# yumi-crew/pose_estimation

Measured on NVIDIA B200. Metric: icp_hypotheses_per_s, higher is better.
Workload: dtype f32

## Files before the change

pose_estimation_b200/csrc/api.cu:

```cuda
#include <algorithm>
#include <cstring>
#include <new>

#include "core_math.cuh"

namespace peb {

int fail(peb_ctx* ctx, int code, const char* fmt, ...) {
  char buf[512];
  va_list ap;
  va_start(ap, fmt);
  vsnprintf(buf, sizeof(buf), fmt, ap);
  va_end(ap);
  if (ctx) ctx->err = buf;
  return code;
}

namespace {

thread_local std::string g_create_error;

__global__ void __launch_bounds__(256) repack_kernel(const unsigned char* __restrict__ raw, size_t stride, int n,
                                                     float w_fill, float4* __restrict__ out) {
  const int i = blockIdx.x * blockDim.x + threadIdx.x;
// ... 202 lines not shown
  if (!strcmp(key, "source_sort_occupancy")) {
    if (value < 1 || value > 1024) return fail(ctx, PEB_E_INVALID_ARG, "source_sort_occupancy out of [1, 1024]");
    ctx->src_sort_occupancy = static_cast<float>(value);
    return PEB_OK;
  }
  if (!strcmp(key, "cert_margin_x1000")) {
    if (value < 0 || value > 4000) return fail(ctx, PEB_E_INVALID_ARG, "cert_margin_x1000 out of [0, 4000]");
    ctx->cert_margin = value / 1000.0f;
    return PEB_OK;
  }
  if (!strcmp(key, "seed_guard_x10")) {
    if (value < 0 || value > 100000) return fail(ctx, PEB_E_INVALID_ARG, "seed_guard_x10 out of [0, 100000]");
    ctx->seed_guard = value / 10.0f;
    return PEB_OK;
  }
  if (!strcmp(key, "batch_streams")) {
    if (value < 0 || value > 32) return fail(ctx, PEB_E_INVALID_ARG, "batch_streams out of [0, 32]");
    ctx->batch_streams = value;
    return PEB_OK;
  }
  if (!strcmp(key, "blocks_factor")) {
    if (value < 0 || value > 4096) return fail(ctx, PEB_E_INVALID_ARG, "blocks_factor out of [0, 4096]");
    ctx->blocks_factor = value;
    return PEB_OK;
  }
  if (!strcmp(key, "coop_max_rows")) {
    if (value < 0 || value > (1 << 20)) return fail(ctx, PEB_E_INVALID_ARG, "coop_max_rows out of [0, 2^20]");
    ctx->coop_max_rows = value;
    return PEB_OK;
  }
  if (!strcmp(key, "blocks_factor_cold")) {
    if (value < 0 || value > 4096) return fail(ctx, PEB_E_INVALID_ARG, "blocks_factor_cold out of [0, 4096]");
    ctx->blocks_factor_cold = value;
    return PEB_OK;
  }
  if (!strcmp(key, "flag_deps")) {
    ctx->flag_deps = value != 0;
    return PEB_OK;
  }
  if (!strcmp(key, "pdl")) {
    ctx->use_pdl = value != 0;
    return PEB_OK;
  }
  if (!strcmp(key, "debug_timers")) {
    ctx->debug_timers = value != 0;
    return PEB_OK;
  }
  if (!strcmp(key, "anchor_seed")) {
    ctx->anchor_seed = value != 0;
    return PEB_OK;
  }
  if (!strcmp(key, "warm_start")) {
    ctx->warm_start = value != 0;
    return PEB_OK;
  }
  if (!strcmp(key, "warm_graph")) {
    if (value < 0 || value > 1) return fail(ctx, PEB_E_INVALID_ARG, "warm_graph must be 0 or 1");
    ctx->warm_graph = value;
    return PEB_OK;
  }
  if (!strcmp(key, "warm_graph_kappa_x100")) {
    if (value < 0 || value > 100000) return fail(ctx, PEB_E_INVALID_ARG, "warm_graph_kappa_x100 out of [0, 100000]");
    ctx->warm_graph_kappa = value / 100.0f;
    return PEB_OK;
  }
  if (!strcmp(key, "warm_graph_queue")) {
// ... 669 lines not shown
```

pose_estimation_b200/csrc/common.cuh:

```cuda
#pragma once

#include <cuda_runtime.h>

#include <cstdarg>
#include <cstdint>
#include <cstdio>
#include <string>
#include <vector>

#include "../../include/pe_b200.h"

#define PEB_HD __host__ __device__ __forceinline__

namespace peb {

constexpr int kSmCount = 148;

struct DevBuf {
  void* p = nullptr;
  size_t cap = 0;
  cudaError_t ensure(size_t bytes) {
    if (bytes <= cap) return cudaSuccess;
    if (p) cudaFree(p);
    p = nullptr;
// ... 56 lines not shown
  bool valid = false;
};

}

struct peb_ctx {
  int device = 0;
  cudaStream_t stream = nullptr;
  std::string err;
  uint64_t launches = 0;
  int nn_group = 1;
  float grid_occupancy = 5.0f;
  bool warm_start = true;
  int warm_upfront = 0;
  int warm_upfront_from = 2;
  int warm_graph = 1;
  float warm_graph_kappa = 0.0f;
  int warm_graph_queue = 0;
  int warm_graph_flat = 1;
  int warm_graph_flat_from = 2, warm_graph_flat_until = 15;
  int warm_graph_peek = 1;
  int cold_graph = 1;
  int warm_graph_min_hyp = 32;
  int warm_bin = 0;
  bool anchor_seed = true;
  int coop_max_rows = 1024;
  float seed_guard = 10.0f;
  int batch_streams = 0;
  std::vector<cudaStream_t> sub_streams;
  std::vector<cudaEvent_t> join_events;
  cudaEvent_t fork_event = nullptr;
  int blocks_factor = 0;
  int blocks_factor_cold = 0;
  bool flag_deps = true;
  peb::DevBuf epochs;
  int* last_err_flag = nullptr;
  bool use_pdl = true;
  bool debug_timers = false;
  peb::DevBuf dbg;
  int dbg_launches = 0;
  peb::DevBuf anchors;
  int nn_cache_from = 0;
  float nn_cache_r = 0.75f;
  peb::DevBuf nn_cache;
  float cert_margin = 0.0f;

  peb::PinnedBuf h_stage;
  peb::PinnedBuf h_small;
  peb::DevBuf d_small;
  peb::DevBuf d_scratch;
  peb::DevBuf sort_scratch;
  peb::DevBuf scan_scratch[4];
  peb::DevBuf d_stage;

  peb::DevBuf tgt_raw;
  peb::DevBuf tgt_nrm_raw;
  size_t n_tgt = 0;
  bool tgt_has_normals = false;
  bool tgt_staged = false;
  cudaEvent_t tgt_stage_event = nullptr;
  peb::Grid tgt_grid;
  peb::DevBuf tgt_knn;
  peb::DevBuf tgt_knn_aux;
  peb::DevBuf tgt_knn_stat;
  bool tgt_knn_valid = false;

// ... 105 lines not shown
```

pose_estimation_b200/csrc/core_math.cuh:

```cuda
#pragma once

#include <cfloat>
#include <cmath>

#include "common.cuh"

namespace peb {

struct Mat4 {
  float m[16];
};

PEB_HD Mat4 mat4_identity() {
  Mat4 a;
#pragma unroll
  for (int i = 0; i < 16; ++i) a.m[i] = (i % 5 == 0) ? 1.0f : 0.0f;
  return a;
}

PEB_HD Mat4 mat4_mul(const Mat4& a, const Mat4& b) {
  Mat4 r;
#pragma unroll
  for (int j = 0; j < 4; ++j)
#pragma unroll
// ... 579 lines not shown
  for (int r = 5; r >= 0; --r) {
    double v = b[r];
    for (int c = r + 1; c < 6; ++c) v -= A[r * 6 + c] * x[c];
    x[r] = v / A[r * 6 + r];
  }
  const double alpha = x[0], beta = x[1], gamma = x[2];
  const double ca = cos(alpha), sa = sin(alpha), cb = cos(beta), sb = sin(beta), cg = cos(gamma), sg = sin(gamma);
  Mat4 T;
  for (int i = 0; i < 16; ++i) T.m[i] = 0.0f;
  T.m[0] = static_cast<float>(cg * cb);
  T.m[4] = static_cast<float>(-sg * ca + cg * sb * sa);
  T.m[8] = static_cast<float>(sg * sa + cg * sb * ca);
  T.m[1] = static_cast<float>(sg * cb);
  T.m[5] = static_cast<float>(cg * ca + sg * sb * sa);
  T.m[9] = static_cast<float>(-cg * sa + sg * sb * ca);
  T.m[2] = static_cast<float>(-sb);
  T.m[6] = static_cast<float>(cb * sa);
  T.m[10] = static_cast<float>(cb * ca);
  T.m[12] = static_cast<float>(x[3]);
  T.m[13] = static_cast<float>(x[4]);
  T.m[14] = static_cast<float>(x[5]);
  T.m[15] = 1.0f;
  return T;
}

struct IcpState {
  Mat4 inc;
  Mat4 final_t;
  double prev_mse, cur_mse;
  double fit_sum;
  int iterations, state, converged, similar;
  int ncorr, active, fit_n, pad0;
  unsigned ticket, ticket_fit;
  int pad1[2];
};

struct IcpCriteria {
  int max_iterations, min_correspondences, max_similar, estimator;
  double rotation_threshold, translation_threshold, mse_rel, mse_abs;
};

PEB_HD void icp_finish_iteration_scripted(IcpState& st, const IcpCriteria& cr, const Mat4& inc, double sum_d2, int n) {
  st.ncorr = n;
  if (n < cr.min_correspondences) {
    st.state = PEB_NO_CORRESPONDENCES;
    st.converged = 0;
    st.active = 0;
    return;
  }
  st.inc = inc;
  st.final_t = mat4_mul(st.inc, st.final_t);
  st.iterations += 1;
  bool is_similar = false;
  bool ret = false;
  int state = PEB_NOT_CONVERGED;
  const float* t = st.inc.m;
  do {
    if (st.iterations >= cr.max_iterations) {
      state = PEB_ITERATIONS;
      ret = true;
      break;
    }
    double cos_angle = 0.5 * static_cast<double>(t[0] + t[5] + t[10] - 1.0f);
    double translation_sqr = static_cast<double>(t[12] * t[12] + t[13] * t[13] + t[14] * t[14]);
    if (cos_angle >= cr.rotation_threshold && translation_sqr <= cr.translation_threshold) {
      if (st.similar >= cr.max_similar) {
        state = PEB_TRANSFORM;
// ... 171 lines not shown
```

pose_estimation_b200/csrc/icp.cu:

```cuda
#include <algorithm>

#include "nn_cache.cuh"
#include "nn_graph.cuh"
#include "nn_search.cuh"
#include "nn_upfront.cuh"

namespace peb {

namespace {

constexpr int kIcpThreads = 128;
constexpr int kMinBlocksSingle = 5;
#ifndef PEB_MIN_BLOCKS_BATCH
#define PEB_MIN_BLOCKS_BATCH 8
#endif
constexpr int kMinBlocksBatch = PEB_MIN_BLOCKS_BATCH;

struct IcpLaunch {
  GridView grid;
  const float4* src;
  float4* work;
  float* slack;
  const int* anchors;
  int n_anchor;
  float seed_guard2;
  int coop_max_rows;
  unsigned long long* dbg;
  int launch_idx;
  IcpState* states;
  double* partials;
  int part_stride;
  int32_t* corr_idx;
  float* corr_d2;
  Mat4* trace;
  peb_icp_result* results;
  IcpCriteria crit;
  double max_dist_sqr;
  double fitness_max_range;
  float stop_d2;
  float fitness_stop_d2;
  float rej_max2;
  int use_rejector;
  int n_src;
  int blocks_per_hyp;
  int trace_cap;
  int fitness_only;
  int warm;
  int* epochs;
  int* err_flag;
// ... 5 lines not shown
  const double* knn_stat;
  float knn_kappa;
  int cold_graph;
  int knn_peek_until;
  const float4* knn_aux;
};

__global__ void icp_init_kernel(IcpState* __restrict__ states, const float* __restrict__ guesses, int H,
                                int* __restrict__ epochs) {
  const int h = blockIdx.x * blockDim.x + threadIdx.x;
  if (epochs && h <= H) epochs[h] = 0;
  if (h >= H) return;
  IcpState st;
  st.inc = mat4_identity();
  if (guesses) {
#pragma unroll
    for (int i = 0; i < 16; ++i) st.final_t.m[i] = guesses[16 * h + i];
  } else {
    st.final_t = mat4_identity();
  }
  st.prev_mse = DBL_MAX;
  st.cur_mse = DBL_MAX;
  st.fit_sum = 0.0;
  st.iterations = 0;
  st.state = PEB_NOT_CONVERGED;
  st.converged = 0;
  st.similar = 0;
  st.ncorr = 0;
  st.active = 1;
  st.fit_n = 0;
  st.pad0 = 0;
  st.ticket = 0;
  st.ticket_fit = 0;
  st.pad1[0] = st.pad1[1] = 0;
  states[h] = st;
}

template <int NACC>
__device__ __forceinline__ double block_reduce_acc(double (&acc)[NACC], double (*sm)[kAccMax]) {
  const int lane = threadIdx.x & 31, warp = threadIdx.x >> 5;
#pragma unroll
  for (int i = 0; i < NACC; ++i) {
    double v = acc[i];
#pragma unroll
    for (int o = 16; o > 0; o >>= 1) v += __shfl_xor_sync(0xFFFFFFFFu, v, o);
    if (lane == 0) sm[warp][i] = v;
  }
  __syncthreads();
  double r = 0.0;
  if (threadIdx.x < NACC) {
#pragma unroll
    for (int w = 0; w < kIcpThreads / 32; ++w) r += sm[w][threadIdx.x];
  }
  return r;
}

template <int NACC>
__device__ __forceinline__ void reduce_partials(const double* __restrict__ part, int n_blocks, double (*sm)[kAccMax],
                                                double* sm_out) {
  const int lane = threadIdx.x & 31, warp = threadIdx.x >> 5;
  constexpr int kW = kIcpThreads / 32;
  double v = 0.0;
  if (lane < NACC) {
    const int per = (n_blocks + kW - 1) / kW;
    const int b0 = warp * per, b1 = min(b0 + per, n_blocks);
    const double* p = part + lane;
    int b = b0;
// ... 50 lines not shown
template <int MB>
__device__ __noinline__ void finish_iteration(IcpState* st, const IcpCriteria* cr, const double* acc, Mat4* trace,
                                              int trace_cap, unsigned long long* dbg) {
  if (dbg) dbg[5] = global_ns();
  IcpState s = *st;
  if (dbg) dbg[6] = global_ns() + (s.iterations < -5 ? 1 : 0);
  icp_finish_iteration(s, *cr, acc);
  if (dbg) dbg[7] = global_ns() + (s.iterations < -5 ? 1 : 0);
  s.ticket = 0;
  if (trace && s.state != PEB_NO_CORRESPONDENCES && s.iterations >= 1 && s.iterations <= trace_cap)
    trace[s.iterations - 1] = s.inc;
  *st = s;
}

__device__ __forceinline__ void pdl_trigger_and_wait() {
  asm volatile("griddepcontrol.launch_dependents;");
  asm volatile("griddepcontrol.wait;" ::: "memory");
}

__device__ __forceinline__ int ld_acquire_gpu(const int* p) {
  int v;
  asm volatile("ld.acquire.gpu.global.s32 %0, [%1];" : "=r"(v) : "l"(p) : "memory");
  return v;
}


constexpr int kEpochStopped = 1 << 20;
constexpr unsigned long long kFlagWaitLimitNs = 20ull * 1000ull * 1000ull * 1000ull;
__device__ __forceinline__ void wait_for_hypothesis(const int* __restrict__ solved, int need, int* err_flag) {
  if (threadIdx.x == 0 && ld_acquire_gpu(solved) < need) {
    const unsigned long long t0 = global_ns();
    unsigned spins = 0;
    while (ld_acquire_gpu(solved) < need) {
      __nanosleep(40);
      if ((++spins & 0xFFFu) == 0u && global_ns() - t0 > kFlagWaitLimitNs) {
        atomicExch(err_flag, 1);
        break;
      }
    }
  }
  __syncthreads();
}

__device__ __forceinline__ bool graph_pays(const IcpLaunch& L, const IcpState* st) {
  if (!L.knn) return false;
  if (L.knn_kappa <= 0.0f) return true;
  const double mse = __ldcg(&st->cur_mse);
  const double cnt = __ldcg(L.knn_stat + 1);
  return cnt > 0.0 && 4.0 * mse * static_cast<double>(L.knn_kappa) * cnt < __ldcg(L.knn_stat);
}

template <int EST, int NACC>
__device__ __forceinline__ void accumulate_pair_impl(const GridView& g, const float4& p, const NnBest& best,
                                                     double (&acc)[NACC]) {
  const float4 t = g.pts[best.j];
  if (EST == PEB_ESTIMATOR_SVD) {
    const double sx = p.x, sy = p.y, sz = p.z, tx = t.x, ty = t.y, tz = t.z;
    acc[0] += 1.0;
    acc[1] += sx;
    acc[2] += sy;
    acc[3] += sz;
    acc[4] += tx;
    acc[5] += ty;
    acc[6] += tz;
    acc[7] = fma(tx, sx, acc[7]);
    acc[8] = fma(tx, sy, acc[8]);
// ... 146 lines not shown
          best.d2 = l2_simple(p.x, p.y, p.z, t.x, t.y, t.z);
          best.idx = __float_as_int(t.w);
          best.j = j_prev;
        } else {
          best = grid_nn_warm_cert(L.grid, p.x, p.y, p.z, j_prev, L.stop_d2, L.margin, &slack);
        }
        *sl = slack;
      } else {
        if (UPF == 4 || UPF == 6) best = graph ? grid_nn_warm_graph(L.grid, L.knn, p.x, p.y, p.z, j_prev, L.stop_d2, kGraphSkipHopeless, L.launch_idx <= L.knn_peek_until, UPF == 6 ? L.knn_aux : nullptr)
                                   : grid_nn_warm(L.grid, p.x, p.y, p.z, j_prev, L.stop_d2);
        else best = UPF ? grid_nn_warm_upfront<(UPF == 3 ? 3 : 2)>(L.grid, p.x, p.y, p.z, j_prev, L.stop_d2)
                        : grid_nn_warm(L.grid, p.x, p.y, p.z, j_prev, L.stop_d2);
      }
    } else {
      best = grid_nn<G>(L.grid, p.x, p.y, p.z, L.stop_d2);
      if (CERT && lane_in_group == 0) *sl = -1.0f;
    }
  }
  if (in && lane_in_group == 0 && (first || valid)) {
    p.w = __int_as_float(best.j);
    work[i] = p;
  }
  bool keep = valid && best.idx >= 0;
  if (keep && static_cast<double>(best.d2) > L.max_dist_sqr) keep = false;
  if (keep && L.use_rejector && !(best.d2 < L.rej_max2)) keep = false;
  if (in && lane_in_group == 0 && L.corr_idx) {
    const int orig = __float_as_int(L.src[i].w);
    L.corr_idx[orig] = keep ? best.idx : -1;
    L.corr_d2[orig] = keep ? best.d2 : 0.0f;
  }
  if (keep && lane_in_group == 0) accumulate_pair<EST>(L.grid, p, best, acc);
}

template <int G, int EST, int MB, bool CERT, bool FIRST, int UPF>
__device__ __forceinline__ void icp_iteration_body(const IcpLaunch& L, const int h, const int blk) {
  unsigned long long t_dbg[5];
  if (L.dbg) t_dbg[0] = global_ns();
  constexpr int NACC = (EST == PEB_ESTIMATOR_SVD) ? kAccSvd : kAccLls;
  __shared__ double sm[kIcpThreads / 32][kAccMax];
  __shared__ double sm_tot[kAccMax];
  __shared__ float s_inc[16];
  __shared__ int s_flags[4];
  __shared__ CoopTile s_tile[kIcpThreads / 32];
  IcpState* st = L.states + h;
  if (threadIdx.x < 16) s_inc[threadIdx.x] = FIRST ? __ldcg(&st->final_t.m[threadIdx.x]) : __ldcg(&st->inc.m[threadIdx.x]);
  if (threadIdx.x == 32) {
    const int active = __ldcg(&st->active);
    const int first = FIRST ? 1 : 0;
    int apply = 1;
    if (first) {
      apply = 0;
      for (int i = 0; i < 16; ++i) {
        const float g = __ldcg(&st->final_t.m[i]);
        if (g != ((i % 5 == 0) ? 1.0f : 0.0f)) apply = 1;
      }
    }
    s_flags[0] = active;
    s_flags[1] = first;
    s_flags[2] = apply;
    const int graph = ((UPF == 4 || UPF == 6) && graph_pays(L, st)) ? 1 : 0;
    s_flags[3] = graph;
  }
  __syncthreads();
  if (!s_flags[0]) return;
  constexpr bool first = FIRST;
  const bool apply = s_flags[2] != 0;
// ... 20 lines not shown
  if (threadIdx.x == 0) {
    const unsigned t = atomicAdd(&st->ticket, 1u);
    s_last = (t == static_cast<unsigned>(L.blocks_per_hyp) - 1u);
  }
  __syncthreads();
  if (!s_last) return;
  __threadfence();
  if (L.dbg) t_dbg[2] = global_ns();
  reduce_partials<NACC>(part, L.blocks_per_hyp, sm, sm_tot);
  if (L.dbg) t_dbg[3] = global_ns();
  if (threadIdx.x == 0) {
    finish_iteration<MB>(st, &L.crit, sm_tot, L.trace, L.trace_cap, (L.dbg && h == 0) ? L.dbg + 8 * L.launch_idx : nullptr);
    if (L.dbg && h == 0) {
      t_dbg[4] = global_ns();
      for (int k = 0; k < 5; ++k) L.dbg[8 * L.launch_idx + k] = t_dbg[k];
    }
    if (L.epochs) {
      const int still_active = st->active;
      __threadfence();
      atomicAdd(L.epochs + h, still_active ? 1 : kEpochStopped);
    }
  }
}

template <int G, int EST, int MB, bool CERT, bool FIRST, int UPF = 0>
__global__ void __launch_bounds__(kIcpThreads, MB) icp_iteration_kernel(const IcpLaunch L) {
  if (FIRST || L.epochs == nullptr) {
    pdl_trigger_and_wait();
  } else {
    asm volatile("griddepcontrol.launch_dependents;");
    wait_for_hypothesis(L.epochs + blockIdx.y, L.launch_idx, L.err_flag);
  }
  icp_iteration_body<G, EST, MB, CERT, FIRST, UPF>(L, blockIdx.y, blockIdx.x);
}

constexpr int kBinQ = 4;
constexpr int kBinTile = kBinQ * kIcpThreads;
constexpr int kBinClasses = 5;

__device__ __forceinline__ int bin_class_of_rows(int rows) {
  return rows >= 7 ? 0 : rows >= 5 ? 1 : rows >= 3 ? 2 : rows == 2 ? 3 : 4;
}

template <int EST, int MB>
__global__ void __launch_bounds__(kIcpThreads, MB) icp_iteration_binned_kernel(const IcpLaunch L) {
  if (L.epochs == nullptr) {
    pdl_trigger_and_wait();
  } else {
    asm volatile("griddepcontrol.launch_dependents;");
    wait_for_hypothesis(L.epochs + blockIdx.y, L.launch_idx, L.err_flag);
  }
  const int h = blockIdx.y, blk = blockIdx.x;
  constexpr int NACC = (EST == PEB_ESTIMATOR_SVD) ? kAccSvd : kAccLls;
  __shared__ double sm[kIcpThreads / 32][kAccMax];
  __shared__ double sm_tot[kAccMax];
  __shared__ float s_inc[16];
  __shared__ int s_active;
  __shared__ float s_qx[kBinTile], s_qy[kBinTile], s_qz[kBinTile], s_d2[kBinTile];
  __shared__ int s_idx[kBinTile], s_j[kBinTile];
  __shared__ unsigned short s_key[kBinTile], s_perm[kBinTile];
  __shared__ int s_cnt[2][kBinClasses + 1];
  IcpState* st = L.states + h;
  if (threadIdx.x < 16) s_inc[threadIdx.x] = __ldcg(&st->inc.m[threadIdx.x]);
  if (threadIdx.x == 32) s_active = __ldcg(&st->active);
  if (threadIdx.x >= 64 && threadIdx.x < 64 + 2 * (kBinClasses + 1)) (&s_cnt[0][0])[threadIdx.x - 64] = 0;
  __syncthreads();
// ... 554 lines not shown
  float4 p = make_float4(0.f, 0.f, 0.f, 0.f);
  if (i < nq) p = q[i];
  const bool valid = i < nq && finite3(p.x, p.y, p.z);
  NnBest best;
  best.d2 = pos_inf();
  best.idx = -1;
  best.j = -1;
  if (valid) best = grid_nn<G>(g, p.x, p.y, p.z, pos_inf());
  if (i < nq && lane_in_group == 0) {
    out_idx[i] = best.idx;
    out_d2[i] = best.d2;
  }
}

float stop_bound(double max_dist_sqr) {
  if (!(max_dist_sqr < static_cast<double>(FLT_MAX))) return INFINITY;
  if (max_dist_sqr < 0.0) return 0.0f;
  float f = static_cast<float>(max_dist_sqr);
  if (static_cast<double>(f) < max_dist_sqr) f = nextafterf(f, INFINITY);
  return f;
}

int prof_mark(peb_ctx* ctx, int slot) {
  if (!ctx->profile) return PEB_OK;
  while (static_cast<int>(ctx->prof_events.size()) <= slot) {
    cudaEvent_t e;
    PEB_CUDA(ctx, cudaEventCreate(&e));
    ctx->prof_events.push_back(e);
  }
  PEB_CUDA(ctx, cudaEventRecord(ctx->prof_events[slot], ctx->stream));
  return PEB_OK;
}

template <int G, bool FIRST>
int launch_one_iteration(peb_ctx* ctx, const IcpLaunch& L, size_t H, int estimator) {
  dim3 grid(L.blocks_per_hyp, static_cast<unsigned>(H));
  constexpr int S = PEB_ESTIMATOR_SVD, P = PEB_ESTIMATOR_POINT_TO_PLANE_LLS;
  const bool cert = G == 1 && L.margin > 0.0f;
  const bool svd = estimator == PEB_ESTIMATOR_SVD;
#define PEB_ICP_LAUNCH(EST, MB, CERT) \
  PEB_LAUNCH_PDL(ctx, (icp_iteration_kernel<G, EST, MB, CERT, FIRST>), grid, dim3(kIcpThreads), L)
  if (G == 1 && !FIRST && !cert && ctx->warm_upfront && L.warm && L.launch_idx >= ctx->warm_upfront_from) {
#define PEB_ICP_LAUNCH_UPF(EST, MB, RW) \
  PEB_LAUNCH_PDL(ctx, (icp_iteration_kernel<1, EST, MB, false, false, RW>), grid, dim3(kIcpThreads), L)
    if (ctx->warm_upfront == 3) {
      if (H == 1) { if (svd) PEB_ICP_LAUNCH_UPF(S, kMinBlocksSingle, 3); else PEB_ICP_LAUNCH_UPF(P, kMinBlocksSingle, 3); }
      else        { if (svd) PEB_ICP_LAUNCH_UPF(S, kMinBlocksBatch, 3);  else PEB_ICP_LAUNCH_UPF(P, kMinBlocksBatch, 3); }
    } else {
      if (H == 1) { if (svd) PEB_ICP_LAUNCH_UPF(S, kMinBlocksSingle, 2); else PEB_ICP_LAUNCH_UPF(P, kMinBlocksSingle, 2); }
      else        { if (svd) PEB_ICP_LAUNCH_UPF(S, kMinBlocksBatch, 2);  else PEB_ICP_LAUNCH_UPF(P, kMinBlocksBatch, 2); }
    }
#undef PEB_ICP_LAUNCH_UPF
    return PEB_OK;
  }
  if (G == 1 && !FIRST && !cert && !L.cache && L.warm && L.knn && H > 1) {
#define PEB_ICP_LAUNCH_GQ(TQ) \
  do { \
    if (svd) PEB_LAUNCH_PDL(ctx, (icp_iteration_graphq_kernel<S, kMinBlocksBatch, TQ>), grid, dim3(kIcpThreads), L); \
    else     PEB_LAUNCH_PDL(ctx, (icp_iteration_graphq_kernel<P, kMinBlocksBatch, TQ>), grid, dim3(kIcpThreads), L); \
  } while (0)
    if (ctx->warm_graph_queue == 8) { PEB_ICP_LAUNCH_GQ(8); return PEB_OK; }
    if (ctx->warm_graph_queue == 16) { PEB_ICP_LAUNCH_GQ(16); return PEB_OK; }
#undef PEB_ICP_LAUNCH_GQ
    if (L.knn_aux && L.launch_idx >= ctx->warm_graph_flat_from && L.launch_idx <= ctx->warm_graph_flat_until) {
      if (svd) PEB_LAUNCH_PDL(ctx, (icp_iteration_kernel<1, S, kMinBlocksBatch, false, false, 6>), grid, dim3(kIcpThreads), L);
      else     PEB_LAUNCH_PDL(ctx, (icp_iteration_kernel<1, P, kMinBlocksBatch, false, false, 6>), grid, dim3(kIcpThreads), L);
      return PEB_OK;
    }
    if (svd) PEB_LAUNCH_PDL(ctx, (icp_iteration_kernel<1, S, kMinBlocksBatch, false, false, 4>), grid, dim3(kIcpThreads), L);
    else     PEB_LAUNCH_PDL(ctx, (icp_iteration_kernel<1, P, kMinBlocksBatch, false, false, 4>), grid, dim3(kIcpThreads), L);
    return PEB_OK;
  }
  if (G == 1 && !FIRST && !cert && !L.cache && L.warm && ctx->warm_bin && H > 1) {
    if (svd) PEB_LAUNCH_PDL(ctx, (icp_iteration_binned_kernel<S, kMinBlocksBatch>), grid, dim3(kIcpThreads), L);
    else     PEB_LAUNCH_PDL(ctx, (icp_iteration_binned_kernel<P, kMinBlocksBatch>), grid, dim3(kIcpThreads), L);
    return PEB_OK;
  }
  if (G == 1 && !FIRST && !cert && L.cache && L.warm) {
#define PEB_ICP_LAUNCH_CACHED(EST, MB) \
  PEB_LAUNCH_PDL(ctx, (icp_iteration_cached_kernel<EST, MB>), grid, dim3(kIcpThreads), L)
    if (H == 1) { if (svd) PEB_ICP_LAUNCH_CACHED(S, kMinBlocksSingle); else PEB_ICP_LAUNCH_CACHED(P, kMinBlocksSingle); }
    else        { if (svd) PEB_ICP_LAUNCH_CACHED(S, kMinBlocksBatch);  else PEB_ICP_LAUNCH_CACHED(P, kMinBlocksBatch); }
#undef PEB_ICP_LAUNCH_CACHED
    return PEB_OK;
  }
  if (H == 1) {
    if (cert) { if (svd) PEB_ICP_LAUNCH(S, kMinBlocksSingle, (G == 1)); else PEB_ICP_LAUNCH(P, kMinBlocksSingle, (G == 1)); }
    else      { if (svd) PEB_ICP_LAUNCH(S, kMinBlocksSingle, false);    else PEB_ICP_LAUNCH(P, kMinBlocksSingle, false); }
  } else {
    if (cert) { if (svd) PEB_ICP_LAUNCH(S, kMinBlocksBatch, (G == 1)); else PEB_ICP_LAUNCH(P, kMinBlocksBatch, (G == 1)); }
    else      { if (svd) PEB_ICP_LAUNCH(S, kMinBlocksBatch, false);    else PEB_ICP_LAUNCH(P, kMinBlocksBatch, false); }
  }
#undef PEB_ICP_LAUNCH
  return PEB_OK;
}

int launch_one_iteration_g(peb_ctx* ctx, int G, bool first, const IcpLaunch& L, size_t H, int estimator) {
#define PEB_ICP_G(GG) return first ? launch_one_iteration<GG, true>(ctx, L, H, estimator) : launch_one_iteration<GG, false>(ctx, L, H, estimator)
  switch (G) {
    case 1: PEB_ICP_G(1);
    case 2: PEB_ICP_G(2);
    case 4: PEB_ICP_G(4);
    case 8: PEB_ICP_G(8);
    case 16: PEB_ICP_G(16);
    default: return fail(ctx, PEB_E_INVALID_ARG, "nn group width %d is not one of 1,2,4,8,16", G);
  }
#undef PEB_ICP_G
}

int launch_fitness_g(peb_ctx* ctx, int G, const IcpLaunch& L, size_t H) {
  dim3 grid(L.blocks_per_hyp, static_cast<unsigned>(H));
  switch (G) {
    case 1: PEB_LAUNCH_PDL(ctx, icp_fitness_kernel<1>, grid, dim3(kIcpThreads), L); break;
    case 2: PEB_LAUNCH_PDL(ctx, icp_fitness_kernel<2>, grid, dim3(kIcpThreads), L); break;
    case 4: PEB_LAUNCH_PDL(ctx, icp_fitness_kernel<4>, grid, dim3(kIcpThreads), L); break;
    case 8: PEB_LAUNCH_PDL(ctx, icp_fitness_kernel<8>, grid, dim3(kIcpThreads), L); break;
    default: PEB_LAUNCH_PDL(ctx, icp_fitness_kernel<16>, grid, dim3(kIcpThreads), L); break;
  }
  return PEB_OK;
}

int blocks_for(int n, size_t H, int G, int factor) {
  if (factor <= 0) factor = H >= 256 ? 32 : 16;
  const int want = ceil_div(std::max(n, 1), kIcpThreads / G);
  int bph;
  if (H == 1)
    bph = std::min(want, kSmCount * 8);
  else
    bph = std::min(want, std::max(1, static_cast<int>((static_cast<size_t>(kSmCount) * factor + H - 1) / H)));
  return std::max(bph, 1);
}
// ... 89 lines not shown
    L.trace_cap = cap;
    ctx->last_trace_cap = cap;
  }
  const int g_cold = ctx->nn_group;
  const int g_warm = ctx->warm_start ? 1 : g_cold;
  const bool per_launch = ctx->profile_level >= 2;
  const int launches = std::max(prm->max_iterations, 1);
  const bool flag_deps = ctx->flag_deps && ctx->use_pdl && !per_launch && !ctx->debug_timers && !single_mode && H >= 16 &&
                         launches < kEpochStopped;
  ctx->last_err_flag = nullptr;
  if (flag_deps) {
    PEB_CUDA(ctx, ctx->epochs.ensure((H + 1) * sizeof(int)));
    L.epochs = ctx->epochs.as<int>();
    L.err_flag = L.epochs + H;
    ctx->last_err_flag = L.err_flag;
  }
  PEB_LAUNCH(ctx, icp_init_kernel, ceil_div(static_cast<long long>(H + 1), 128), 128, 0, L.states, d_guesses,
             static_cast<int>(H), L.epochs);
  if (L.margin > 0.0f)
    PEB_CUDA(ctx, cudaMemsetAsync(L.slack, 0xFF, std::max<size_t>(H * static_cast<size_t>(n), 1) * sizeof(float), ctx->stream));
  IcpLaunch Lc = L, Lw = L;
  Lc.blocks_per_hyp = blocks_for(n, H, g_cold, cold_blocks_factor(ctx));
  Lc.warm = 0;
  if (ctx->warm_start && ctx->anchor_seed && g_cold == 1 && n >= 64 && H * static_cast<size_t>(n) >= (1u << 20) && H <= 65535) {
    const int n_anchor = ceil_div(n, 32);
    PEB_CUDA(ctx, ctx->anchors.ensure(H * static_cast<size_t>(n_anchor) * sizeof(int)));
    Lc.n_anchor = n_anchor;
    dim3 agrid(ceil_div(n_anchor, 128), static_cast<unsigned>(H));
    PEB_LAUNCH(ctx, icp_anchor_kernel, agrid, 128, 0, Lc, ctx->anchors.as<int>());
    Lc.anchors = ctx->anchors.as<int>();
  }
  Lw.blocks_per_hyp = blocks_for(n, H, g_warm, ctx->blocks_factor);
  Lw.warm = ctx->warm_start ? 1 : 0;
  if (ctx->warm_graph && ctx->warm_start && g_warm == 1 && !single_mode && !(L.margin > 0.0f) && !ctx->warm_upfront &&
      !ctx->warm_bin && ctx->nn_cache_from == 0 && H >= static_cast<size_t>(ctx->warm_graph_min_hyp) && launches > 1) {
    PEB_TRY(target_graph_ensure(ctx));
    Lw.knn = ctx->tgt_knn.as<KnnRow>();
    Lw.knn_stat = ctx->tgt_knn_stat.as<double>();
    Lw.knn_kappa = ctx->warm_graph_kappa;
    Lw.knn_peek_until = ctx->warm_graph_peek;
    Lw.knn_aux = ctx->warm_graph_flat ? ctx->tgt_knn_aux.as<float4>() : nullptr;
    if (ctx->cold_graph && Lc.anchors) {
      Lc.knn = Lw.knn;
      Lc.cold_graph = 1;
    }
  }
  const int cache_from = (ctx->nn_cache_from > 0 && ctx->warm_start && g_warm == 1 && !(L.margin > 0.0f)) ? ctx->nn_cache_from : 0;
  NnCache* cache_buf = nullptr;
  if (cache_from > 0 && cache_from < launches) {
    PEB_CUDA(ctx, ctx->nn_cache.ensure(H * static_cast<size_t>(std::max(n, 1)) * sizeof(NnCache)));
    cache_buf = ctx->nn_cache.as<NnCache>();
    Lw.cache_r_cells = ctx->nn_cache_r;
  }
  auto set_cache = [&](int it) {
    Lw.cache = (cache_buf && it >= cache_from && it < launches) ? cache_buf : nullptr;
    Lw.cache_init = it == cache_from ? 1 : 0;
  };
  ctx->prof_launches = 0;
  ctx->prof_chain_ends = 0;
  if (ctx->debug_timers) {
    PEB_CUDA(ctx, ctx->dbg.ensure(static_cast<size_t>(launches) * 8 * sizeof(unsigned long long)));
    PEB_CUDA(ctx, cudaMemsetAsync(ctx->dbg.p, 0, static_cast<size_t>(launches) * 8 * sizeof(unsigned long long), ctx->stream));
    Lc.dbg = Lw.dbg = ctx->dbg.as<unsigned long long>();
    ctx->dbg_launches = launches;
  }

  int S = 1;
  if (!single_mode && !per_launch && !ctx->debug_timers) {
    const size_t want = ctx->batch_streams > 0 ? ctx->batch_streams : (H >= 512 ? 4 : 2);
    S = static_cast<int>(std::min<size_t>(want, H / 16));
    S = std::max<int>(S, static_cast<int>((H + 32767) / 32768));
  }
  if (S <= 1 && H > 65535)
    return fail(ctx, PEB_E_UNSUPPORTED, "align_batch: %zu hypotheses in one launch (profile level 2 / debug timers "
                "allow at most 65535)", H);
  if (S > 1) {
    PEB_TRY(ensure_sub_streams(ctx, S));
    PEB_TRY(prof_mark(ctx, 0));
    PEB_CUDA(ctx, cudaEventRecord(ctx->fork_event, ctx->stream));
    const size_t per = (H + S - 1) / S;
    struct StreamSwap {
      peb_ctx* c;
      cudaStream_t keep;
      StreamSwap(peb_ctx* c_, cudaStream_t s) : c(c_), keep(c_->stream) { c->stream = s; }
      ~StreamSwap() { c->stream = keep; }
    };
    auto chunk_of = [&](const IcpLaunch& base, size_t h0) {
      IcpLaunch C = base;
      C.states += h0;
      C.work += h0 * static_cast<size_t>(n);
      C.slack += h0 * static_cast<size_t>(n);
      C.partials += h0 * static_cast<size_t>(base.part_stride) * kAccMax;
      C.results += h0;
      if (C.anchors) C.anchors += h0 * static_cast<size_t>(C.n_anchor);
      if (C.epochs) C.epochs += h0;
      if (C.cache) C.cache += h0 * static_cast<size_t>(n);
      return C;
    };
    for (int c = 0; c < S; ++c) PEB_CUDA(ctx, cudaStreamWaitEvent(ctx->sub_streams[c], ctx->fork_event, 0));
    for (int it = 0; it <= launches; ++it) {
      for (int c = 0; c < S; ++c) {
        const size_t h0 = c * per, h1 = std::min(H, h0 + per);
        if (h0 >= h1) continue;
        StreamSwap swap(ctx, ctx->sub_streams[c]);
        Lc.launch_idx = Lw.launch_idx = it;
        set_cache(it);
        if (it == 0) {
          PEB_TRY(launch_one_iteration_g(ctx, g_cold, true, chunk_of(Lc, h0), h1 - h0, prm->estimator));
        } else if (it < launches) {
          PEB_TRY(launch_one_iteration_g(ctx, g_warm, false, chunk_of(Lw, h0), h1 - h0, prm->estimator));
        } else {
          PEB_TRY(prof_mark(ctx, 2 + c));
          PEB_TRY(launch_fitness_g(ctx, g_warm, chunk_of(Lw, h0), h1 - h0));
          PEB_CUDA(ctx, cudaEventRecord(ctx->join_events[c], ctx->stream));
        }
      }
    }
    for (int c = 0; c < S; ++c) PEB_CUDA(ctx, cudaStreamWaitEvent(ctx->stream, ctx->join_events[c], 0));
    if (ctx->profile) {
      ctx->prof_launches = 1;
      ctx->prof_span_launches = launches;
      ctx->prof_chain_ends = static_cast<int>(std::min<size_t>(S, (H + per - 1) / per));
    }
    return PEB_OK;
  }

  if (!per_launch) PEB_TRY(prof_mark(ctx, 0));
  for (int it = 0; it < launches; ++it) {
    if (per_launch) PEB_TRY(prof_mark(ctx, 2 * it));
    Lc.launch_idx = Lw.launch_idx = it;
    set_cache(it);
    if (it == 0)
      PEB_TRY(launch_one_iteration_g(ctx, g_cold, true, Lc, H, prm->estimator));
    else
      PEB_TRY(launch_one_iteration_g(ctx, g_warm, false, Lw, H, prm->estimator));
    if (per_launch) PEB_TRY(prof_mark(ctx, 2 * it + 1));
  }
  Lw.launch_idx = launches;
  set_cache(launches);
  if (per_launch) {
    PEB_TRY(prof_mark(ctx, 2 * launches));
    PEB_TRY(launch_fitness_g(ctx, g_warm, Lw, H));
    PEB_TRY(prof_mark(ctx, 2 * launches + 1));
    if (ctx->profile) ctx->prof_launches = launches + 1;
  } else {
    PEB_TRY(prof_mark(ctx, 1));
    PEB_TRY(launch_fitness_g(ctx, g_warm, Lw, H));
    if (ctx->profile) {
      ctx->prof_launches = 1;
      ctx->prof_span_launches = launches;
    }
  }
  return PEB_OK;
}

#ifdef PEB_COOP_STATS
extern "C" __attribute__((visibility("default"))) int peb_debug_coop_stats(unsigned long long* out8, int reset) {
  if (cudaMemcpyFromSymbol(out8, g_coop_stats, 8 * sizeof(unsigned long long)) != cudaSuccess) return -1;
  if (reset) {
    unsigned long long z[8] = {};
    cudaMemcpyToSymbol(g_coop_stats, z, sizeof(z));
  }
  return 0;
}
#endif

int fitness_device(peb_ctx* ctx, const float* d_T, double max_range, peb_icp_result* d_result) {
  if (!ctx->tgt_grid.valid) return fail(ctx, PEB_E_NO_TARGET, "fitness_score: no target set (peb_target_set)");
// ... 38 lines not shown
```

Baseline: 16900.

## Split ICP iteration into separate search and moment-accumulation kernels for batches

For batches of at least split_min_hyp hypotheses, each ICP iteration now runs two kernels instead of one fused kernel. A search kernel finds nearest neighbours and writes the indices into the work buffer. A moment kernel then reads those indices back, accumulates the estimator moments, reduces them and finishes the iteration. The search kernel gets its own occupancy bound and block count, and the two are linked by per-hypothesis searched counters and flag waits. This decouples the register-heavy double-precision accumulation from the divergent grid search, at the cost of an extra launch, a second pass over the work buffer and more spin-wait synchronisation.

```diff
diff --git a/pose_estimation_b200/csrc/api.cu b/pose_estimation_b200/csrc/api.cu
--- a/pose_estimation_b200/csrc/api.cu
+++ b/pose_estimation_b200/csrc/api.cu
@@ -258,6 +258,21 @@
   if (!strcmp(key, "blocks_factor_cold")) {
     if (value < 0 || value > 4096) return fail(ctx, PEB_E_INVALID_ARG, "blocks_factor_cold out of [0, 4096]");
     ctx->blocks_factor_cold = value;
+    return PEB_OK;
+  }
+  if (!strcmp(key, "blocks_factor_search")) {
+    if (value < 0 || value > 4096) return fail(ctx, PEB_E_INVALID_ARG, "blocks_factor_search out of [0, 4096]");
+    ctx->blocks_factor_search = value;
+    return PEB_OK;
+  }
+  if (!strcmp(key, "split_moments")) {
+    if (value < 0 || value > 1) return fail(ctx, PEB_E_INVALID_ARG, "split_moments must be 0 or 1");
+    ctx->split_moments = value;
+    return PEB_OK;
+  }
+  if (!strcmp(key, "split_min_hyp")) {
+    if (value < 2) return fail(ctx, PEB_E_INVALID_ARG, "split_min_hyp must be >= 2 (batches only)");
+    ctx->split_min_hyp = value;
     return PEB_OK;
   }
   if (!strcmp(key, "flag_deps")) {
diff --git a/pose_estimation_b200/csrc/common.cuh b/pose_estimation_b200/csrc/common.cuh
--- a/pose_estimation_b200/csrc/common.cuh
+++ b/pose_estimation_b200/csrc/common.cuh
@@ -112,6 +112,9 @@
   cudaEvent_t fork_event = nullptr;
   int blocks_factor = 0;
   int blocks_factor_cold = 0;
+  int blocks_factor_search = 0;
+  int split_moments = 1;
+  int split_min_hyp = 256;
   bool flag_deps = true;
   peb::DevBuf epochs;
   int* last_err_flag = nullptr;
diff --git a/pose_estimation_b200/csrc/core_math.cuh b/pose_estimation_b200/csrc/core_math.cuh
--- a/pose_estimation_b200/csrc/core_math.cuh
+++ b/pose_estimation_b200/csrc/core_math.cuh
@@ -635,7 +635,8 @@
   int iterations, state, converged, similar;
   int ncorr, active, fit_n, pad0;
   unsigned ticket, ticket_fit;
-  int pad1[2];
+  unsigned ticket_search;
+  int searched;
 };
 
 struct IcpCriteria {
diff --git a/pose_estimation_b200/csrc/icp.cu b/pose_estimation_b200/csrc/icp.cu
--- a/pose_estimation_b200/csrc/icp.cu
+++ b/pose_estimation_b200/csrc/icp.cu
@@ -15,6 +15,10 @@
 #define PEB_MIN_BLOCKS_BATCH 8
 #endif
 constexpr int kMinBlocksBatch = PEB_MIN_BLOCKS_BATCH;
+#ifndef PEB_MIN_BLOCKS_SEARCH
+#define PEB_MIN_BLOCKS_SEARCH 10
+#endif
+constexpr int kMinBlocksSearch = PEB_MIN_BLOCKS_SEARCH;
 
 struct IcpLaunch {
   GridView grid;
@@ -86,7 +90,8 @@
   st.pad0 = 0;
   st.ticket = 0;
   st.ticket_fit = 0;
-  st.pad1[0] = st.pad1[1] = 0;
+  st.ticket_search = 0;
+  st.searched = 0;
   states[h] = st;
 }
 
@@ -203,6 +208,22 @@
     const unsigned long long t0 = global_ns();
     unsigned spins = 0;
     while (ld_acquire_gpu(solved) < need) {
+      __nanosleep(40);
+      if ((++spins & 0xFFFu) == 0u && global_ns() - t0 > kFlagWaitLimitNs) {
+        atomicExch(err_flag, 1);
+        break;
+      }
+    }
+  }
+  __syncthreads();
+}
+
+__device__ __forceinline__ void wait_for_search(const int* __restrict__ searched, int need, const int* __restrict__ solved,
+                                                int* err_flag) {
+  if (threadIdx.x == 0 && ld_acquire_gpu(searched) < need && ld_acquire_gpu(solved) < kEpochStopped) {
+    const unsigned long long t0 = global_ns();
+    unsigned spins = 0;
+    while (ld_acquire_gpu(searched) < need && ld_acquire_gpu(solved) < kEpochStopped) {
       __nanosleep(40);
       if ((++spins & 0xFFFu) == 0u && global_ns() - t0 > kFlagWaitLimitNs) {
         atomicExch(err_flag, 1);
@@ -415,6 +436,73 @@
   if (keep && lane_in_group == 0) accumulate_pair<EST>(L.grid, p, best, acc);
 }
 
+template <int UPF>
+__device__ __forceinline__ NnBest icp_search_query(const IcpLaunch& L, const int h, float4* __restrict__ work, const int i,
+                                                   const bool first, const bool apply, const bool graph, const float* T,
+                                                   CoopTile* tile, float4& p, bool& valid) {
+  const bool in = i < L.n_src;
+  p = make_float4(0.f, 0.f, 0.f, 1.f);
+  if (in) p = first ? L.src[i] : work[i];
+  const int j_prev = first ? -1 : __float_as_int(p.w);
+  valid = in && finite3(p.x, p.y, p.z);
+  if (valid && apply) {
+    float ox, oy, oz;
+    transform_icp(T, p.x, p.y, p.z, ox, oy, oz);
+    p.x = ox;
+    p.y = oy;
+    p.z = oz;
+  }
+  NnBest best;
+  best.d2 = pos_inf();
+  best.idx = -1;
+  best.j = -1;
+  if (first && L.anchors) {
+    best = first_iteration_search(L, h, i, valid, p, T, apply, tile);
+  } else if (valid) {
+    if (L.warm && j_prev >= 0 && j_prev < L.grid.n) {
+      if (UPF == 4 || UPF == 6) best = graph ? grid_nn_warm_graph(L.grid, L.knn, p.x, p.y, p.z, j_prev, L.stop_d2, kGraphSkipHopeless, L.launch_idx <= L.knn_peek_until, UPF == 6 ? L.knn_aux : nullptr)
+                                 : grid_nn_warm(L.grid, p.x, p.y, p.z, j_prev, L.stop_d2);
+      else best = grid_nn_warm(L.grid, p.x, p.y, p.z, j_prev, L.stop_d2);
+    } else {
+      best = grid_nn<1>(L.grid, p.x, p.y, p.z, L.stop_d2);
+    }
+  }
+  if (in && (first || valid)) {
+    p.w = __int_as_float(best.j);
+    work[i] = p;
+  }
+  return best;
+}
+
+__device__ __forceinline__ bool keep_pair(const IcpLaunch& L, const bool valid, const NnBest& best) {
+  bool keep = valid && best.idx >= 0;
+  if (keep && static_cast<double>(best.d2) > L.max_dist_sqr) keep = false;
+  if (keep && L.use_rejector && !(best.d2 < L.rej_max2)) keep = false;
+  return keep;
+}
+
+template <bool FIRST, int UPF>
+__device__ __forceinline__ void load_launch_flags(const IcpLaunch& L, const IcpState* st, float* s_inc, int* s_flags) {
+  if (threadIdx.x < 16) s_inc[threadIdx.x] = FIRST ? __ldcg(&st->final_t.m[threadIdx.x]) : __ldcg(&st->inc.m[threadIdx.x]);
+  if (threadIdx.x == 32) {
+    const int active = __ldcg(&st->active);
+    const int first = FIRST ? 1 : 0;
+    int apply = 1;
+    if (first) {
+      apply = 0;
+      for (int i = 0; i < 16; ++i) {
+        const float g = __ldcg(&st->final_t.m[i]);
+        if (g != ((i % 5 == 0) ? 1.0f : 0.0f)) apply = 1;
+      }
+    }
+    s_flags[0] = active;
+    s_flags[1] = first;
+    s_flags[2] = apply;
+    const int graph = ((UPF == 4 || UPF == 6) && graph_pays(L, st)) ? 1 : 0;
+    s_flags[3] = graph;
+  }
+}
+
 template <int G, int EST, int MB, bool CERT, bool FIRST, int UPF>
 __device__ __forceinline__ void icp_iteration_body(const IcpLaunch& L, const int h, const int blk) {
   unsigned long long t_dbg[5];
@@ -501,6 +589,111 @@
     wait_for_hypothesis(L.epochs + blockIdx.y, L.launch_idx, L.err_flag);
   }
   icp_iteration_body<G, EST, MB, CERT, FIRST, UPF>(L, blockIdx.y, blockIdx.x);
+}
+
+template <int MB, bool FIRST, int UPF>
+__global__ void __launch_bounds__(kIcpThreads, MB) icp_search_kernel(const IcpLaunch L) {
+  if (FIRST || L.epochs == nullptr) {
+    pdl_trigger_and_wait();
+  } else {
+    asm volatile("griddepcontrol.launch_dependents;");
+    wait_for_hypothesis(L.epochs + blockIdx.y, L.launch_idx, L.err_flag);
+  }
+  const int h = blockIdx.y, blk = blockIdx.x;
+  __shared__ float s_inc[16];
+  __shared__ int s_flags[4];
+  __shared__ CoopTile s_tile[kIcpThreads / 32];
+  IcpState* st = L.states + h;
+  load_launch_flags<FIRST, UPF>(L, st, s_inc, s_flags);
+  __syncthreads();
+  if (s_flags[0]) {
+    const bool apply = s_flags[2] != 0;
+    const bool graph = (UPF == 4 || UPF == 6) && s_flags[3] != 0;
+    float4* work = L.work + static_cast<size_t>(h) * L.n_src;
+    for (int base = blk * kIcpThreads; base < L.n_src; base += gridDim.x * kIcpThreads) {
+      const int i = base + threadIdx.x;
+      float4 p;
+      bool valid;
+      const NnBest best = icp_search_query<UPF>(L, h, work, i, FIRST, apply, graph, s_inc, &s_tile[threadIdx.x >> 5], p, valid);
+      int* w = reinterpret_cast<int*>(work + i) + 3;
+      if (valid && best.j >= 0 && !finite3(p.x, p.y, p.z)) *w = -2 - best.j;
+      else if (!FIRST && !valid && i < L.n_src && __float_as_int(p.w) <= -2) *w = -1;
+    }
+  }
+  if (L.epochs && s_flags[0]) {
+    __syncthreads();
+    if (threadIdx.x == 0) {
+      __threadfence();
+      if (atomicAdd(&st->ticket_search, 1u) == gridDim.x - 1u) {
+        st->ticket_search = 0u;
+        __threadfence();
+        atomicAdd(&st->searched, 1);
+      }
+    }
+  }
+}
+
+template <int EST, int MB>
+__global__ void __launch_bounds__(kIcpThreads, MB) icp_moment_kernel(const IcpLaunch L) {
+  if (L.epochs == nullptr) {
+    pdl_trigger_and_wait();
+  } else {
+    asm volatile("griddepcontrol.launch_dependents;");
+    wait_for_search(&L.states[blockIdx.y].searched, L.launch_idx + 1, L.epochs + blockIdx.y, L.err_flag);
+  }
+  const int h = blockIdx.y, blk = blockIdx.x;
+  constexpr int NACC = (EST == PEB_ESTIMATOR_SVD) ? kAccSvd : kAccLls;
+  __shared__ double sm[kIcpThreads / 32][kAccMax];
+  __shared__ double sm_tot[kAccMax];
+  __shared__ int s_active;
+  IcpState* st = L.states + h;
+  if (threadIdx.x == 0) s_active = __ldcg(&st->active);
+  __syncthreads();
+  if (!s_active) return;
+
+  double acc[NACC];
+#pragma unroll
+  for (int i = 0; i < NACC; ++i) acc[i] = 0.0;
+  const float4* work = L.work + static_cast<size_t>(h) * L.n_src;
+  for (int i = blk * kIcpThreads + threadIdx.x; i < L.n_src; i += L.blocks_per_hyp * kIcpThreads) {
+    const float4 p = __ldcg(work + i);
+    bool valid = finite3(p.x, p.y, p.z);
+    int j = __float_as_int(p.w);
+    if (j <= -2) {
+      valid = true;
+      j = -2 - j;
+    }
+    if (!valid || j < 0) continue;
+    const float4 t = L.grid.pts[j];
+    NnBest best;
+    best.d2 = l2_simple(p.x, p.y, p.z, t.x, t.y, t.z);
+    best.idx = point_index(t);
+    best.j = j;
+    if (keep_pair(L, valid, best)) accumulate_pair<EST>(L.grid, p, best, acc);
+  }
+
+  const double r = block_reduce_acc<NACC>(acc, sm);
+  double* part = L.partials + (static_cast<size_t>(h) * L.part_stride) * kAccMax;
+  if (threadIdx.x < NACC) __stcg(part + static_cast<size_t>(blk) * kAccMax + threadIdx.x, r);
+  __threadfence();
+  __syncthreads();
+  __shared__ int s_last;
+  if (threadIdx.x == 0) {
+    const unsigned t = atomicAdd(&st->ticket, 1u);
+    s_last = (t == static_cast<unsigned>(L.blocks_per_hyp) - 1u);
+  }
+  __syncthreads();
+  if (!s_last) return;
+  __threadfence();
+  reduce_partials<NACC>(part, L.blocks_per_hyp, sm, sm_tot);
+  if (threadIdx.x == 0) {
+    finish_iteration<MB>(st, &L.crit, sm_tot, L.trace, L.trace_cap, nullptr);
+    if (L.epochs) {
+      const int still_active = st->active;
+      __threadfence();
+      atomicAdd(L.epochs + h, still_active ? 1 : kEpochStopped);
+    }
+  }
 }
 
 constexpr int kBinQ = 4;
@@ -1121,8 +1314,37 @@
   return PEB_OK;
 }
 
+bool split_iteration(const peb_ctx* ctx, const IcpLaunch& L, size_t H, int G, bool first) {
+  if (!ctx->split_moments || H < static_cast<size_t>(ctx->split_min_hyp) || H <= 1 || G != 1 || L.margin > 0.0f || L.dbg ||
+      L.corr_idx)
+    return false;
+  if (first) return true;
+  if (L.cache || (ctx->warm_upfront && L.warm && L.launch_idx >= ctx->warm_upfront_from)) return false;
+  if (L.warm && L.knn) return ctx->warm_graph_queue == 0;
+  return !(L.warm && ctx->warm_bin);
+}
+
+template <bool FIRST>
+int launch_split_iteration(peb_ctx* ctx, const IcpLaunch& L, size_t H, int estimator, int search_bph) {
+  const dim3 sgrid(search_bph, static_cast<unsigned>(H)), mgrid(L.blocks_per_hyp, static_cast<unsigned>(H));
+  if (FIRST)
+    PEB_LAUNCH_PDL(ctx, (icp_search_kernel<kMinBlocksBatch, true, 0>), sgrid, dim3(kIcpThreads), L);
+  else if (L.warm && L.knn && L.knn_aux && L.launch_idx >= ctx->warm_graph_flat_from && L.launch_idx <= ctx->warm_graph_flat_until)
+    PEB_LAUNCH_PDL(ctx, (icp_search_kernel<kMinBlocksSearch, false, 6>), sgrid, dim3(kIcpThreads), L);
+  else if (L.warm && L.knn)
+    PEB_LAUNCH_PDL(ctx, (icp_search_kernel<kMinBlocksSearch, false, 4>), sgrid, dim3(kIcpThreads), L);
+  else
+    PEB_LAUNCH_PDL(ctx, (icp_search_kernel<kMinBlocksSearch, false, 0>), sgrid, dim3(kIcpThreads), L);
+  if (estimator == PEB_ESTIMATOR_SVD)
+    PEB_LAUNCH_PDL(ctx, (icp_moment_kernel<PEB_ESTIMATOR_SVD, kMinBlocksBatch>), mgrid, dim3(kIcpThreads), L);
+  else
+    PEB_LAUNCH_PDL(ctx, (icp_moment_kernel<PEB_ESTIMATOR_POINT_TO_PLANE_LLS, kMinBlocksBatch>), mgrid, dim3(kIcpThreads), L);
+  return PEB_OK;
+}
+
 template <int G, bool FIRST>
-int launch_one_iteration(peb_ctx* ctx, const IcpLaunch& L, size_t H, int estimator) {
+int launch_one_iteration(peb_ctx* ctx, const IcpLaunch& L, size_t H, int estimator, int search_bph) {
+  if (G == 1 && search_bph > 0) return launch_split_iteration<FIRST>(ctx, L, H, estimator, search_bph);
   dim3 grid(L.blocks_per_hyp, static_cast<unsigned>(H));
   constexpr int S = PEB_ESTIMATOR_SVD, P = PEB_ESTIMATOR_POINT_TO_PLANE_LLS;
   const bool cert = G == 1 && L.margin > 0.0f;
@@ -1184,8 +1406,8 @@
   return PEB_OK;
 }
 
-int launch_one_iteration_g(peb_ctx* ctx, int G, bool first, const IcpLaunch& L, size_t H, int estimator) {
-#define PEB_ICP_G(GG) return first ? launch_one_iteration<GG, true>(ctx, L, H, estimator) : launch_one_iteration<GG, false>(ctx, L, H, estimator)
+int launch_one_iteration_g(peb_ctx* ctx, int G, bool first, const IcpLaunch& L, size_t H, int estimator, int search_bph) {
+#define PEB_ICP_G(GG) return first ? launch_one_iteration<GG, true>(ctx, L, H, estimator, search_bph) : launch_one_iteration<GG, false>(ctx, L, H, estimator, search_bph)
   switch (G) {
     case 1: PEB_ICP_G(1);
     case 2: PEB_ICP_G(2);
@@ -1341,6 +1563,9 @@
   }
   Lw.blocks_per_hyp = blocks_for(n, H, g_warm, ctx->blocks_factor);
   Lw.warm = ctx->warm_start ? 1 : 0;
+  const int fs = ctx->blocks_factor_search;
+  const int search_bph_cold = blocks_for(n, H, 1, fs > 0 ? fs : cold_blocks_factor(ctx));
+  const int search_bph_warm = blocks_for(n, H, 1, fs > 0 ? fs : ctx->blocks_factor);
   if (ctx->warm_graph && ctx->warm_start && g_warm == 1 && !single_mode && !(L.margin > 0.0f) && !ctx->warm_upfront &&
       !ctx->warm_bin && ctx->nn_cache_from == 0 && H >= static_cast<size_t>(ctx->warm_graph_min_hyp) && launches > 1) {
     PEB_TRY(target_graph_ensure(ctx));
@@ -1364,6 +1589,11 @@
   auto set_cache = [&](int it) {
     Lw.cache = (cache_buf && it >= cache_from && it < launches) ? cache_buf : nullptr;
     Lw.cache_init = it == cache_from ? 1 : 0;
+  };
+  bool split_prefix = true;
+  auto split_bph = [&](int it) {
+    split_prefix = split_prefix && split_iteration(ctx, it == 0 ? Lc : Lw, H, it == 0 ? g_cold : g_warm, it == 0);
+    return split_prefix ? (it == 0 ? search_bph_cold : search_bph_warm) : 0;
   };
   ctx->prof_launches = 0;
   ctx->prof_chain_ends = 0;
@@ -1408,16 +1638,17 @@
     };
     for (int c = 0; c < S; ++c) PEB_CUDA(ctx, cudaStreamWaitEvent(ctx->sub_streams[c], ctx->fork_event, 0));
     for (int it = 0; it <= launches; ++it) {
+      Lc.launch_idx = Lw.launch_idx = it;
+      set_cache(it);
+      const int sb = it < launches ? split_bph(it) : 0;
       for (int c = 0; c < S; ++c) {
         const size_t h0 = c * per, h1 = std::min(H, h0 + per);
         if (h0 >= h1) continue;
         StreamSwap swap(ctx, ctx->sub_streams[c]);
-        Lc.launch_idx = Lw.launch_idx = it;
-        set_cache(it);
         if (it == 0) {
-          PEB_TRY(launch_one_iteration_g(ctx, g_cold, true, chunk_of(Lc, h0), h1 - h0, prm->estimator));
+          PEB_TRY(launch_one_iteration_g(ctx, g_cold, true, chunk_of(Lc, h0), h1 - h0, prm->estimator, sb));
         } else if (it < launches) {
-          PEB_TRY(launch_one_iteration_g(ctx, g_warm, false, chunk_of(Lw, h0), h1 - h0, prm->estimator));
+          PEB_TRY(launch_one_iteration_g(ctx, g_warm, false, chunk_of(Lw, h0), h1 - h0, prm->estimator, sb));
         } else {
           PEB_TRY(prof_mark(ctx, 2 + c));
           PEB_TRY(launch_fitness_g(ctx, g_warm, chunk_of(Lw, h0), h1 - h0));
@@ -1439,10 +1670,11 @@
     if (per_launch) PEB_TRY(prof_mark(ctx, 2 * it));
     Lc.launch_idx = Lw.launch_idx = it;
     set_cache(it);
+    const int sb = split_bph(it);
     if (it == 0)
-      PEB_TRY(launch_one_iteration_g(ctx, g_cold, true, Lc, H, prm->estimator));
+      PEB_TRY(launch_one_iteration_g(ctx, g_cold, true, Lc, H, prm->estimator, sb));
     else
-      PEB_TRY(launch_one_iteration_g(ctx, g_warm, false, Lw, H, prm->estimator));
+      PEB_TRY(launch_one_iteration_g(ctx, g_warm, false, Lw, H, prm->estimator, sb));
     if (per_launch) PEB_TRY(prof_mark(ctx, 2 * it + 1));
   }
   Lw.launch_idx = launches;
```

Result: faster. 17800 (median of 6 runs) (+5.3%).
